# lucidrains/glom-pytorch

Hardware: NVIDIA H100
Metric: column-iterations/sec (BxNxLxiters) at dim=512 L=6 224/14 (higher is better)
Workload: dtype bf16

## Files before the change

### glom_pytorch_b200/csrc/engine.h

```cpp
#pragma once
#include <cuda.h>
#include <cuda_runtime.h>
#include <cuda_bf16.h>
#include <stdarg.h>
#include <stddef.h>
#include <stdint.h>
#include <stdio.h>
#include <atomic>
#include <mutex>
#include <vector>

#include "../../include/glom_b200.h"

namespace glom {

enum ProfKind { PROF_ATTN = 0, PROF_GEMM1 = 1, PROF_GEMM2 = 2, PROF_PREP = 3, PROF_TOKENIZE = 4, PROF_KINDS = 5 };
struct Profiler {
  bool enabled = false;
  std::vector<cudaEvent_t> ev;
  size_t used = 0;
  struct Span { int kind; size_t a, b; };
  std::vector<Span> spans;
  size_t mark(cudaStream_t st) {
    if (used == ev.size()) { cudaEvent_t e; cudaEventCreate(&e); ev.push_back(e); }
// ... 14 lines not shown
  int rows;
  int G;
  int hidden;
  int attend_self, mask_side, mask_d2_max;
  int bn2;
  int part_w;
  int nparts;
};

struct PackedLayout {
  size_t w1_off, w2_off, b1_off, b2_off, total;
};
PackedLayout packed_layout(int d, int L, int precision);

struct WorkspaceLayout {
  size_t s32_off;
  size_t s32_bytes;
  size_t sb_off[2];
  size_t sp_off[2];
  size_t xb_off;
  size_t h_off;
  size_t h_bytes;
  size_t c_off;
  size_t c_bytes;
  size_t nsq_off[2];
  size_t nsq_bytes;
  size_t attn_acc_off;
  size_t attn_acc_bytes;
  size_t total;
};
WorkspaceLayout workspace_layout(const Geometry& g, int precision, int iters, int return_all);

struct SettleLayout {
  WorkspaceLayout fwd;
  size_t dsq_off;
  size_t flags_off;
  size_t frozen_off;
  size_t block_frozen_off;
  size_t done_off;
  size_t level_q_off;
  size_t flags_bytes;
  size_t total;
};
SettleLayout settle_layout(const Geometry& g, int max_iters, int return_all = 0);

struct QueueLayout {
  SettleLayout settle;
  size_t slab_off[2];
  size_t queue_off;
  size_t slot_img_off;
  size_t age_off;
  size_t pending_off;
  size_t gather_off;
  size_t fresh_off;
  size_t block_fresh_off;
  size_t head_off;
  size_t unfinished_off;
  size_t queue_bytes;
  size_t total;
};
QueueLayout queue_layout(const Geometry& g, int max_iters);

struct QueueSlots {
  int *slot_img, *age, *pending, *gather_img, *fresh, *block_fresh, *head, *unfinished;
  int images, frames, max_iters;
};

struct Bf16Buffers {
  const float* s32_in;  float* s32_out;
  int s32_in_bcast;
  const __nv_bfloat16* sb_in;  __nv_bfloat16* sb_out;
  const __nv_bfloat16* sp_in;  __nv_bfloat16* sp_out;
  const __nv_bfloat16* xb;
  __nv_bfloat16* h;  __nv_bfloat16* c;
  float* attn_acc;
  const float* nsq_in;  float* nsq_out;
  const float* pos;
  const __nv_bfloat16* w1;  const __nv_bfloat16* w2;  const float* b1;  const float* b2;
  const int* frozen;
  const int* block_frozen;
  float* dsq_out;
  const int* block_fresh;
  int ii_reduce;
};

static inline int rep_h_blocks(int n) {
  int a = n, b = 128;
  while (b) { const int r = a % b; a = b; b = r; }
  return n / a;
}
static inline int rep_row_blocks(int n) { return (rep_h_blocks(n) * 128 + 255) / 256; }

typedef CUresult (*EncodeTiledFn)(CUtensorMap*, CUtensorMapDataType, cuuint32_t, void*, const cuuint64_t*,
                                  const cuuint64_t*, const cuuint32_t*, const cuuint32_t*, CUtensorMapInterleave,
                                  CUtensorMapSwizzle, CUtensorMapL2promotion, CUtensorMapFloatOOBfill);

struct Launch {
  EncodeTiledFn enc; int num_sms; cudaStream_t st; Profiler* prof;
  int launches;
  char err[400];
  int launched(cudaError_t e, const char* what = nullptr) { ++launches; return check(e, what); }
  int launched(const char* what = nullptr) { return launched(cudaGetLastError(), what); }
  int check(cudaError_t e, const char* what = nullptr) {
    if (e == cudaSuccess) return 0;
    return what ? fail(GLOM_B200_ERR_CUDA, "%s: %s", what, cudaGetErrorString(e)) : fail(GLOM_B200_ERR_CUDA, "%s", cudaGetErrorString(e));
  }
  int fail(int code, const char* fmt, ...) {
    char msg[sizeof(err)];
    va_list ap;
    va_start(ap, fmt);
    vsnprintf(msg, sizeof(msg), fmt, ap);
    va_end(ap);
    snprintf(err, sizeof(err), "%s", msg);
    return code;
  }
};
#define GLOM_TRY(x) do { if (const int r_ = (x)) return r_; } while (0)

int launch_prep(const Geometry& g, const float* state_in, const float* init_levels, const float* pos, const float* tokens,
                float* s32_dst, __nv_bfloat16* sb, __nv_bfloat16* sp, __nv_bfloat16* xb, float* nsq, Launch& ln);

int step_bf16(const Geometry& g, const Bf16Buffers& b, int step_index, Launch& ln);

int launch_settle_converge(const Geometry& g, int step, float tol, const float* dsq, const float* nsq, int* frozen,
                           int* block_frozen, unsigned int* done, float* level_q, int32_t* steps, Launch& ln,
                           const QueueSlots* q = nullptr);
int launch_queue_init(const Geometry& g, const QueueSlots& q, int* frozen, int* block_frozen, unsigned int* done, Launch& ln);
int launch_queue_schedule(const Geometry& g, const QueueSlots& q, int admit, int* frozen, int* block_frozen, Launch& ln);
int launch_queue_fill(const Geometry& g, const QueueSlots& q, const float* tokens, const float* pos, const float* state_in,
                      const float* init_levels, float* state_out, float* slab, __nv_bfloat16* sb, __nv_bfloat16* sp,
                      float* nsq, __nv_bfloat16* xb, Launch& ln);
int launch_settle_gather(const Geometry& g, int max_iters, const int32_t* steps, const float* slab, float* state_out,
                         const float* s0, int s0_bcast, Launch& ln);
int launch_steps_schedule(const Geometry& g, int t, int max_steps, const int32_t* steps, int* frozen, int* block_frozen,
                          Launch& ln);
int launch_steps_fill(const Geometry& g, int max_steps, const int32_t* steps, float* states, Launch& ln);
int launch_level_fill(const Geometry& g, float* states, Launch& ln);

constexpr int kAttnF32Queries = 16;
constexpr int kAttnF32MaxDimPlusN = (int)((227 * 1024) / (kAttnF32Queries * sizeof(float)));

struct F32Buffers {
  const float* s_in;  float* s_out;
  const float* x;  const float* pos;
  float* h;  float* c;
  const float* w1;  const float* w2;  const float* b1;  const float* b2;
};
int step_f32(const Geometry& g, const F32Buffers& b, Launch& ln);
int launch_broadcast_init(const Geometry& g, const float* state_in, const float* init_levels, float* dst, Launch& ln);

int launch_pack(int d, int L, int precision, const float* bu_w1, const float* bu_b1, const float* bu_w2, const float* bu_b2,
                const float* td_w1, const float* td_b1, const float* td_w2, const float* td_b2, void* packed, Launch& ln);

int launch_tokenize(const float* img, const float* w, const float* bias, float* tokens, int B, int H, int W, int p, int d,
                    Launch& ln);

int launch_islands(const float* states, int slabs, int side_h, int side_w, int L, int d, float threshold, float* cos_right,
                   float* cos_down, float* agreement, int* labels, int* num_islands, Launch& ln);
int launch_island_tree(const int* labels, const float* states, int slabs, int n, int L, int d, int* size, int* parent,
                       float* containment, float* nested, float* embedding, float* member_cos, float* coherence,
                       Launch& ln);

cudaError_t launch_clock_probe(unsigned long long* out, unsigned long long spin_ns, cudaStream_t st);
cudaError_t tc_kernel_clocks(unsigned long long* out , bool reset);

int launch_patchify_bf16(const float* img, const float* w, __nv_bfloat16* patches, __nv_bfloat16* wtok, int B, int H, int W,
// ... 106 lines not shown
```

### glom_pytorch_b200/csrc/gemm_sched.cuh

```cuda
#pragma once
#include "tc_common.cuh"

namespace glom {

struct GemmParams {
  int rows, d, L, n, G;
  int num_m, num_n, num_tiles;
  int m128;
  int z0;
  int n_half;
  const float* bias;
  const float* s32_in;
  int s_bcast;
  const __nv_bfloat16* c_in;
  const float* pos;
  float* s32_out;
  __nv_bfloat16* sb_out;
  __nv_bfloat16* sp_out;
  float* nsq_out;
  int nparts;
  float* tok_out;
  int tok_kb;
  const int* frozen;
  const int* block_frozen;
  float* dsq_out;
  const int* block_fresh;
  int num_m_rep, num_full_tiles;
  unsigned long long full_mask, rep_mask;
  int remap_l, h_period;
};

struct TileInfo {
  int z;
  int m_blk, n_blk;
  int num_kb;
};

__host__ __device__ __forceinline__ int nth_set_bit(unsigned long long m, int k) {
  int z = 0;
  for (;; ++z)
    if ((m >> z) & 1ull) { if (k == 0) return z; --k; }
}

template <int MODE, bool REDUCED = false>
__host__ __device__ __forceinline__ TileInfo decode_tile(const GemmParams& p, int tile) {
  TileInfo t;
  if (REDUCED && p.num_m_rep > 0) {
    const bool full = tile < p.num_full_tiles;
    const int nm = full ? p.num_m : p.num_m_rep;
    const int r = full ? tile / p.num_n : (tile - p.num_full_tiles) / p.num_n;
    t.n_blk = tile % p.num_n;
    t.m_blk = r % nm;
    t.z = nth_set_bit(full ? p.full_mask : p.rep_mask, r / nm);
  } else {
    t.n_blk = tile % p.num_n;
    const int r = tile / p.num_n;
    t.m_blk = r % p.num_m;
    t.z = p.z0 + r / p.num_m;
  }
  if (MODE == 0) t.num_kb = p.d / BK;
  else if (MODE == 1) t.num_kb = ((t.z == p.L - 1) ? 4 * p.d : 8 * p.d) / BK;
  else t.num_kb = p.tok_kb;
  return t;
}

template <int MODE>
__host__ __device__ __forceinline__ int sched_tile(const GemmParams& p, int c, int C, int it) {
  if (MODE != 1) { const int t = c + it * C; return t < p.num_tiles ? t : -1; }
  const int S = p.n_half;
  const int B = p.num_tiles - S;
  const int heavy = B % C;
  const int nb = (B - c + C - 1) / C;
  const int nbig = nb > 0 ? nb : 0;
  if (it < nbig) return c + it * C;
  int k = it - nbig;
  const int light = C - heavy;
  const int first = (2 * light < S) ? 2 * light : S;
  if (c >= heavy) {
    if (k < 2) { const int j = k * light + (c - heavy); if (j < first) return B + j; }
    k -= 2;
    if (k < 0) return -1;
  }
  const int j = first + k * C + c;
  return j < S ? B + j : -1;
}

__host__ __device__ __forceinline__ bool ii_k1_full(int z, int t) { return (z & 1) ? z <= 2 * t - 3 : z <= 2 * t; }
__host__ __device__ __forceinline__ bool ii_k2_full(int l, int t) { return l <= t; }
__host__ __device__ __forceinline__ int ii_k3_full_levels(int t) { return t; }

template <typename Full>
__host__ __forceinline__ void set_reduced(GemmParams& p, int z_end, int num_m_rep, Full full) {
  p.num_m_rep = num_m_rep;
  p.full_mask = p.rep_mask = 0;
  for (int z = p.z0; z < z_end; ++z) (full(z) ? p.full_mask : p.rep_mask) |= 1ull << z;
  p.num_full_tiles = __builtin_popcountll(p.full_mask) * p.num_m * p.num_n;
  p.num_tiles = p.num_full_tiles + __builtin_popcountll(p.rep_mask) * num_m_rep * p.num_n;
}

__host__ __device__ __forceinline__ void attn_item(int it, int full_items, int per_img, int ntiles, int l_full, int& b, int& l) {
  if (it >= full_items) { b = 0; l = l_full + (it - full_items) / ntiles; }
  else { b = it / per_img; l = (it % per_img) / ntiles; }
}

}
```

### glom_pytorch_b200/csrc/glom_api.cu

```cuda
#include "../../include/glom_b200.h"
#include "../../include/glom_b200_tree.h"
#include "engine.h"

#include <mutex>
#include <stdarg.h>
#include <stdio.h>
#include <string.h>

namespace glom {

static thread_local char g_err[512] = "";
static thread_local Profiler g_prof;
static thread_local Launch g_launch{};

static int fail(int code, const char* fmt, ...) {
  va_list ap;
  va_start(ap, fmt);
  vsnprintf(g_err, sizeof(g_err), fmt, ap);
  va_end(ap);
  return code;
}

static bool misaligned(const void* p, size_t a) { return reinterpret_cast<uintptr_t>(p) % a != 0; }

// ... 253 lines not shown
static void set_parity(StepBuffers& s, int p) {
  s.step.sb_in = s.sb[p]; s.step.sb_out = s.sb[p ^ 1];
  s.step.sp_in = s.sp[p]; s.step.sp_out = s.sp[p ^ 1];
  s.step.nsq_in = s.nsq[p]; s.step.nsq_out = s.nsq[p ^ 1];
}

struct SettleFlags { int *frozen, *block_frozen; float* dsq; unsigned int* done; float* level_q; };
static SettleFlags bind_settle_flags(const SettleLayout& sl, void* workspace) {
  char* ws = static_cast<char*>(workspace);
  return {reinterpret_cast<int*>(ws + sl.frozen_off), reinterpret_cast<int*>(ws + sl.block_frozen_off),
          reinterpret_cast<float*>(ws + sl.dsq_off), reinterpret_cast<unsigned int*>(ws + sl.done_off),
          reinterpret_cast<float*>(ws + sl.level_q_off)};
}

struct SettleRun { float tol; int32_t* steps; };

struct ForwardArgs {
  const glom_b200_cfg* cfg; const void* packed_weights; const float *tokens, *pos, *state_in, *init_levels; float* state_out;
  int batch, iters, return_all; void* workspace; size_t workspace_bytes; void* stream;
  int resume_parity = -1;
  const SettleRun* settle = nullptr;
  const int32_t* steps = nullptr;
};

static int forward_impl(const ForwardArgs& a) {
  const glom_b200_cfg* cfg = a.cfg;
  const float *state_in = a.state_in, *init_levels = a.init_levels;
  float* state_out = a.state_out;
  const int iters = a.iters, return_all = a.return_all;
  const SettleRun* settle = a.settle;
  const int32_t* steps = a.steps;
  if (int r = check_cfg(cfg)) return r;
  if (a.batch < 1 || iters < 0) return fail(GLOM_B200_ERR_INVALID, "batch must be >= 1 and iters >= 0");
  if (cfg->precision == GLOM_B200_FP32 && cfg->dim + cfg->n > kAttnF32MaxDimPlusN)
    return fail(GLOM_B200_ERR_INVALID,
                "fp32 consensus keeps %d (dim + n) floats per block in shared memory: dim + n must be <= %d (got %d)",
                kAttnF32Queries, kAttnF32MaxDimPlusN, cfg->dim + cfg->n);
  if (int r = check_tensors("", true, a.packed_weights, a.tokens, a.pos, state_in, init_levels, state_out, a.workspace)) return r;
  DeviceInfo di{};
  if (int r = device_info(&di)) return r;
  const Geometry g = make_geometry(cfg, a.batch);
  const bool freeze = settle || steps;
  const SettleLayout sl = freeze ? settle_layout(g, iters, return_all) : SettleLayout{};
  const WorkspaceLayout wl = freeze ? sl.fwd : workspace_layout(g, cfg->precision, iters, return_all);
  const size_t ws_need = freeze ? sl.total : wl.total;
  if (!a.workspace || a.workspace_bytes < ws_need)
    return fail(GLOM_B200_ERR_WORKSPACE, "workspace: need %zu bytes, got %zu", ws_need, a.workspace_bytes);
  const PackedLayout pl = packed_layout(g.d, g.L, cfg->precision);
  char* ws = static_cast<char*>(a.workspace);
  Launch& ln = begin_launch(di.sms, a.stream);
  const size_t slab = (size_t)g.rows * g.L * g.d;

  float* wslab = reinterpret_cast<float*>(ws + wl.s32_off);
  auto loc = [&](int t) -> float* {
    if (return_all) return state_out + (size_t)t * slab;
    return ((iters - t) % 2 == 0) ? state_out : wslab;
  };

  if (cfg->precision == GLOM_B200_BF16) {
    StepBuffers sbuf = bind_step_buffers(wl, pl, a.workspace, a.packed_weights, a.pos);
    Bf16Buffers& b = sbuf.step;
    const bool resume = a.resume_parity >= 0;
    const int p0 = resume ? a.resume_parity : 0;
    const bool s0_direct = resume || (!return_all && iters >= 1);
    int prep;
    if (resume) {
      prep = launch_prep(g, nullptr, nullptr, a.pos, a.tokens, nullptr, nullptr, nullptr, sbuf.xb, nullptr, ln);
      if (prep == 0 && return_all)
        prep = ln.launched(cudaMemcpyAsync(state_out, state_in, slab * sizeof(float), cudaMemcpyDeviceToDevice, ln.st));
    } else {
      prep = launch_prep(g, state_in, init_levels, a.pos, a.tokens, s0_direct ? nullptr : loc(0), sbuf.sb[0], sbuf.sp[0], sbuf.xb,
                         sbuf.nsq[0], ln);
    }
    if (prep) return fail(prep, "prep launch: %s", ln.err);
    const SettleFlags fl = freeze ? bind_settle_flags(sl, a.workspace) : SettleFlags{};
    b.frozen = fl.frozen; b.block_frozen = fl.block_frozen;
    b.dsq_out = settle ? fl.dsq : nullptr;
    if (settle) {
      if (int r = ln.check(cudaMemsetAsync(ws + sl.flags_off, 0, sl.flags_bytes, ln.st)))
        return fail(r, "settle flags memset: %s", ln.err);
    }
    const bool ii = !state_in && !resume && !freeze && iters >= g.L + 1 && g.L <= 32 &&
                    rep_row_blocks(g.n) < (g.rows + 255) / 256 && (size_t)g.n * g.L * g.d < (1u << 31);
    for (int t = 0; t < iters; ++t) {
      if (steps) {
        if (int r = launch_steps_schedule(g, t, iters, steps, fl.frozen, fl.block_frozen, ln))
          return fail(r, "step schedule launch before step %d: %s", t, ln.err);
      }
      b.s32_in = (s0_direct && t == 0) ? (state_in ? state_in : init_levels) : loc(t); b.s32_out = loc(t + 1);
      b.s32_in_bcast = (s0_direct && t == 0 && !state_in) ? 1 : 0;
      set_parity(sbuf, (t + p0) & 1);
      b.ii_reduce = ii && t < g.L;
      if (int r = step_bf16(g, b, t, ln)) return fail(r, "step %d: %s", t, ln.err);
      if (settle) {
        if (int r = launch_settle_converge(g, t + 1, settle->tol, fl.dsq, b.nsq_out, fl.frozen, fl.block_frozen, fl.done,
                                           fl.level_q, settle->steps, ln))
          return fail(r, "settle convergence launch after step %d: %s", t, ln.err);
      }
    }
    const int32_t* image_steps = settle ? settle->steps : steps;
    if (ii && return_all) {
      if (int r = launch_level_fill(g, state_out, ln)) return fail(r, "return_all level fill launch: %s", ln.err);
    }
    if (image_steps && return_all) {
      if (int r = launch_steps_fill(g, iters, image_steps, state_out, ln)) return fail(r, "return_all fill launch: %s", ln.err);
    } else if (image_steps && iters > 0) {
      if (int r = launch_settle_gather(g, iters, image_steps, wslab, state_out, state_in ? state_in : init_levels,
                                       state_in ? 0 : 1, ln))
        return fail(r, "%s gather launch: %s", settle ? "settle" : "step", ln.err);
    }
  } else {
    const char* pw = static_cast<const char*>(a.packed_weights);
    if (int r = launch_broadcast_init(g, state_in, init_levels, loc(0), ln)) return fail(r, "init launch: %s", ln.err);
    for (int t = 0; t < iters; ++t) {
      F32Buffers b{};
      b.s_in = loc(t); b.s_out = loc(t + 1);
      b.x = a.tokens; b.pos = a.pos;
      b.h = reinterpret_cast<float*>(ws + wl.h_off);
      b.c = reinterpret_cast<float*>(ws + wl.c_off);
      b.w1 = reinterpret_cast<const float*>(pw + pl.w1_off);
      b.w2 = reinterpret_cast<const float*>(pw + pl.w2_off);
      b.b1 = reinterpret_cast<const float*>(pw + pl.b1_off);
      b.b2 = reinterpret_cast<const float*>(pw + pl.b2_off);
      if (int r = step_f32(g, b, ln)) return fail(r, "fp32 step %d launch: %s", t, ln.err);
    }
  }
  g_err[0] = 0;
  return 0;
}

struct FreezeMode { const char* name; const char* bound; int min_bound; };
static const FreezeMode kSettle{"settle", "max_iters", 1}, kForwardSteps{"forward_steps", "max_steps", 0};

static int check_freeze(const FreezeMode& m, const glom_b200_cfg* cfg, int batch, int bound) {
  if (int r = check_cfg(cfg)) return r;
  if (cfg->precision != GLOM_B200_BF16) return fail(GLOM_B200_ERR_INVALID, "%s: bf16 engine only (precision fp32 given)", m.name);
  if (batch < 1) return fail(GLOM_B200_ERR_INVALID, "%s: batch must be >= 1 (got %d)", m.name, batch);
  if (bound < m.min_bound) return fail(GLOM_B200_ERR_INVALID, "%s: %s must be >= %d (got %d)", m.name, m.bound, m.min_bound, bound);
  return 0;
}

static int freeze_workspace_bytes(const FreezeMode& m, const glom_b200_cfg* cfg, int batch, int bound, int return_all,
                                  size_t* out_bytes) {
  if (int r = check_freeze(m, cfg, batch, bound)) return r;
  if (!out_bytes) return fail(GLOM_B200_ERR_INVALID, "out_bytes is NULL");
  *out_bytes = settle_layout(make_geometry(cfg, batch), bound, return_all ? 1 : 0).total;
  return 0;
}

static int check_steps_ptr(const char* fn, const char* arg, const int32_t* steps) {
  if (!steps) return fail(GLOM_B200_ERR_INVALID, "%s: %s is NULL", fn, arg);
  if (misaligned(steps, 4)) return fail(GLOM_B200_ERR_INVALID, "%s: %s must be 4-byte aligned", fn, arg);
  return 0;
}

static int settle_impl(ForwardArgs a, float tol, int32_t* steps_out) {
  if (int r = check_freeze(kSettle, a.cfg, a.batch, a.iters)) return r;
  if (tol != tol) return fail(GLOM_B200_ERR_INVALID, "settle: tol is NaN");
  if (int r = check_steps_ptr("settle", "steps_out", steps_out)) return r;
  const SettleRun run{tol, steps_out};
  a.settle = &run;
  return forward_impl(a);
}

GLOM_B200_API int glom_b200_settle_workspace_bytes(const glom_b200_cfg* cfg, int batch, int max_iters, size_t* out_bytes) {
  return freeze_workspace_bytes(kSettle, cfg, batch, max_iters, 0, out_bytes);
}

GLOM_B200_API int glom_b200_settle_workspace_offset(const glom_b200_cfg* cfg, int batch, int max_iters, int return_all,
                                                    int which, size_t* out_offset, size_t* out_bytes) {
  if (int r = check_freeze(kSettle, cfg, batch, max_iters)) return r;
  if (!out_offset || !out_bytes) return fail(GLOM_B200_ERR_INVALID, "settle: out_offset / out_bytes is NULL");
  const Geometry g = make_geometry(cfg, batch);
  const SettleLayout s = settle_layout(g, max_iters, return_all ? 1 : 0);
  switch (which) {
// ... 527 lines not shown
```

### glom_pytorch_b200/csrc/tc_kernels.cu

```cuda
#include "gemm_sched.cuh"
#include "tc_common.cuh"

#include <stdio.h>
#include <stdlib.h>
#include <string.h>

#include <type_traits>

namespace glom {

constexpr int GEMM_CONSUMER_WARPS = 8;
constexpr int GEMM_THREADS = 128 + 32 * GEMM_CONSUMER_WARPS;
constexpr uint32_t GEMM_PRODUCER_REGS = 40;
constexpr uint32_t GEMM_CONSUMER_REGS = 232;

__device__ unsigned long long g_kernel_clk[PROF_KINDS][8];


template <int MODE, int BN>
struct GemmCfg {
  static constexpr int PARTS = (BN == 256) ? 4 : 2;
  static constexpr int PART_COLS = BN / PARTS;
  static constexpr int THREADS = GEMM_THREADS;
  static constexpr uint32_t B_STAGE_BYTES = BN * BK * 2;
  static constexpr uint32_t STAGE_BYTES = A_STAGE_BYTES + B_STAGE_BYTES;
  static_assert(MODE >= 0 && MODE <= 2, "0 = GEMM1+GELU, 1 = GEMM2+combine, 2 = tokeniser");
  static constexpr int STAGES = (BN == 256) ? 3 : (BN == 128) ? 4 : 5;
  static constexpr uint32_t OUT_BOX_BYTES = 64 * BK * 2;
  static constexpr uint32_t PATCH_BYTES = 4096;
  static constexpr size_t EPI_BYTES = (MODE == 0) ? 2 * (BN / 64) * (size_t)OUT_BOX_BYTES
                                                  : 4 * (size_t)STG_BYTES + (size_t)GEMM_CONSUMER_WARPS * PATCH_BYTES + 4 * 32 * 4;
  static constexpr size_t SMEM_BYTES = 1024  + (size_t)STAGES * STAGE_BYTES + EPI_BYTES + 256 ;
  static_assert(SMEM_BYTES <= 232448, "over the 227 KB of shared memory a block may opt in to");
};

__device__ __forceinline__ void tok_chunk(const uint32_t (&v)[32], const float4 b4, uint8_t* patch, float* dst,
                                          size_t pitch, int lane, int rows_left) {
#pragma unroll
  for (int c = 0; c < 8; ++c)
    *reinterpret_cast<uint4*>(patch + lane * 128 + ((c ^ (lane & 7)) << 4)) =
        make_uint4(v[4 * c], v[4 * c + 1], v[4 * c + 2], v[4 * c + 3]);
  __syncwarp();
  const int c = lane & 7, rsub = lane >> 3;
#pragma unroll
  for (int i = 0; i < 8; ++i) {
    const int r = i * 4 + rsub;
    const float4 a = *reinterpret_cast<const float4*>(patch + r * 128 + ((c ^ (r & 7)) << 4));
    if (r < rows_left)
      *reinterpret_cast<float4*>(dst + (size_t)r * pitch + c * 4) = make_float4(a.x + b4.x, a.y + b4.y, a.z + b4.z, a.w + b4.w);
  }
  __syncwarp();
}

template <int MODE>
__device__ __forceinline__ bool settle_skip(const GemmParams& p, const TileInfo& t) {
  if (p.block_frozen[t.m_blk]) return true;
  return MODE == 0 && t.z == 0 && p.block_fresh != nullptr && !p.block_fresh[t.m_blk];
}

template <int MODE, int BN, bool CNT, bool SETTLE = false>
__global__ void __launch_bounds__(GEMM_THREADS, 1)
gemm_kernel(const __grid_constant__ CUtensorMap map_a0,
            const __grid_constant__ CUtensorMap map_a1,
            const __grid_constant__ CUtensorMap map_a2,
            const __grid_constant__ CUtensorMap map_b,
            const __grid_constant__ CUtensorMap map_out,
            const GemmParams p) {
  using Cfg = GemmCfg<MODE, BN>;
  constexpr int STAGES = Cfg::STAGES;
  constexpr bool RED = MODE != 2 && !SETTLE;
  extern __shared__ uint8_t smem_raw[];
  uint8_t* smem = smem_raw + ((1024u - (smem_u32(smem_raw) & 1023u)) & 1023u);
  uint8_t* epi = smem + (size_t)STAGES * Cfg::STAGE_BYTES;
  float* stg_all = reinterpret_cast<float*>(epi);
  uint8_t* patches = epi + 4 * STG_BYTES;
  float* xch = reinterpret_cast<float*>(patches + (size_t)GEMM_CONSUMER_WARPS * Cfg::PATCH_BYTES);
  uint64_t* full_bar = reinterpret_cast<uint64_t*>(epi + Cfg::EPI_BYTES);
  uint64_t* empty_bar = full_bar + STAGES;

  const int warp = threadIdx.x >> 5;
  const int lane = threadIdx.x & 31;
  constexpr int W_TMA = 0;
  constexpr int W_CONSUMER0 = 4;
  const int cta_rank = (int)(blockIdx.x & 1);
  const int cluster_id = blockIdx.x >> 1;
  const int num_clusters = gridDim.x >> 1;

  if (warp == W_TMA && lane == 0) {
    tma_prefetch_desc(&map_a0);
    tma_prefetch_desc(&map_b);
    if (MODE == 0) { tma_prefetch_desc(&map_a1); tma_prefetch_desc(&map_a2); tma_prefetch_desc(&map_out); }
    for (int i = 0; i < STAGES; ++i) { mbar_init(&full_bar[i], 1); mbar_init(&empty_bar[i], 2 * GEMM_CONSUMER_WARPS); }
    fence_barrier_init();
  }
  cluster_sync_all();
  pdl_launch_dependents();
  pdl_wait();
  const bool clk_thread = blockIdx.x == 0 && warp == W_TMA && lane == 0;
  ClockSample* clk_s = reinterpret_cast<ClockSample*>(empty_bar + STAGES);
  if (clk_thread) *clk_s = clock_sample_begin();
  const bool cnt_cta = CNT && blockIdx.x == 0;
  unsigned long long* const cnt = g_kernel_clk[MODE == 0 ? PROF_GEMM1 : MODE == 1 ? PROF_GEMM2 : PROF_TOKENIZE];
  unsigned long long w0 = 0, w1 = 0;
#define GLOM_CNT_WAIT(acc, stmt) do { if (cnt_cta) { const long long t_ = clock64(); stmt; acc += (unsigned long long)(clock64() - t_); } else { stmt; } } while (0)

  if (warp < W_CONSUMER0) {
    setmaxnreg_dec<GEMM_PRODUCER_REGS>();
    if (warp == W_TMA) {
      const uint32_t elected = elect_one();
      int stage = 0; uint32_t phase = 0;
      const uint32_t smem0 = smem_u32(smem);
      const uint64_t pol_first = l2_policy_evict_first();
      const int kbg_n = 4 * p.d / BK;
      const int blk_skip = (p.m128 - 1) * kbg_n;
      for (int it = 0, tile; (tile = sched_tile<MODE>(p, cluster_id, num_clusters, it)) >= 0; ++it) {
        const TileInfo t = decode_tile<MODE, RED>(p, tile);
        if constexpr (SETTLE) { if (settle_skip<MODE>(p, t)) continue; }
        const CUtensorMap* amap;
        int a_col, b_row;
        if (MODE == 0) {
          const int l = t.z >> 1;
          if (t.z == 0) { amap = &map_a0; a_col = 0; }
          else if (t.z & 1) { amap = &map_a2; a_col = l * p.d; }
          else { amap = &map_a1; a_col = (l - 1) * p.d; }
          b_row = t.z * 4 * p.d + t.n_blk * BN;
        } else if (MODE == 1) {
          amap = &map_a0; a_col = 0;
          b_row = t.z * p.d + t.n_blk * BN;
        } else {
          amap = &map_a0; a_col = 0;
          b_row = t.n_blk * BN;
        }
        const int a_row = t.m_blk * 256 + cta_rank * BM;
        const int blk0 = (2 * t.z * p.m128 + (a_row >> 7)) * kbg_n;
        int td_skip = blk_skip;
        if constexpr (RED && MODE == 1) {
          if (p.num_m_rep > 0 && t.z + 1 >= p.remap_l) td_skip -= ((a_row >> 7) - (a_row >> 7) % p.h_period) * kbg_n;
        }
        for (int kb = 0; kb < t.num_kb; ++kb) {
          GLOM_CNT_WAIT(w0, mbar_wait(&empty_bar[stage], phase ^ 1));
          if (elected) {
            const uint32_t sa = smem0 + (uint32_t)stage * Cfg::STAGE_BYTES;
            uint64_t* bar = &full_bar[stage];
            mbar_arrive_expect_tx(bar, Cfg::STAGE_BYTES);
            if (MODE == 1) {
              const int blk = blk0 + kb + (kb >= kbg_n ? td_skip : 0);
              tma_load_2d_hint(sa, amap, bar, 0, blk * BM, pol_first);
            } else {
              tma_load_2d(sa, amap, bar, a_col + kb * BK, a_row);
            }
            const uint32_t b_half = (uint32_t)cta_rank * (BN / 2);
            tma_load_2d_multicast(sa + A_STAGE_BYTES + b_half * BK * 2, &map_b, bar, kb * BK, b_row + (int)b_half, 0x3);
          }
          __syncwarp();
          if (++stage == STAGES) { stage = 0; phase ^= 1; }
        }
      }
      if (cnt_cta && elected) atomicAdd(&cnt[4], w0);
    }
  } else {
    setmaxnreg_inc<GEMM_CONSUMER_REGS>();
    const int cw = warp - W_CONSUMER0;
    const int wg = cw >> 2, wi = cw & 3;
    const int pair = cw >> 1, x = cw & 1;
    float* stg = stg_all + pair * (STG_BYTES / 4);
    uint8_t* patch = patches + (size_t)cw * Cfg::PATCH_BYTES;
    float* xch_p = xch + pair * 32;
    const uint32_t smem0 = smem_u32(smem);
    const uint64_t pol_stream = l2_policy_evict_first();
    const bool st_issuer = (threadIdx.x & 127) == 0;
    const uint32_t out_wg = smem_u32(epi) + (uint32_t)wg * (BN / 64) * Cfg::OUT_BOX_BYTES;
    const uint32_t st_row = (uint32_t)(16 * wi + 8 * ((lane >> 3) & 1) + (lane & 7)) * 128;
    const int st_jx = lane >> 4, st_sw = lane & 7;
    const uint32_t empty_peer = mapa_shared(smem_u32(empty_bar), (uint32_t)cta_rank ^ 1u);
    auto release = [&](int slot) {
      __syncwarp();
      if (lane == 0) { mbar_arrive(&empty_bar[slot]); mbar_arrive_cluster(empty_peer + 8u * (uint32_t)slot); }
    };
    int stage = 0; uint32_t phase = 0;
    float acc[BN / 2];
    for (int it = 0, tile; (tile = sched_tile<MODE>(p, cluster_id, num_clusters, it)) >= 0; ++it) {
      const TileInfo t = decode_tile<MODE, RED>(p, tile);
      if constexpr (SETTLE) { if (settle_skip<MODE>(p, t)) continue; }
      const int row0 = t.m_blk * 256 + cta_rank * BM + pair * 32;
      const int rows_left = p.rows - row0;
      uint32_t live = ~0u;
      if constexpr (SETTLE && MODE == 1)
        live = __ballot_sync(0xffffffffu, row0 + lane < p.rows && !p.frozen[(row0 + lane) / p.n]);
      bool remap = false;
      if constexpr (RED && MODE == 1) remap = p.num_m_rep > 0 && t.z >= p.remap_l;
      if (MODE == 1 && lane < rows_left) {
        const int src_row = remap ? (row0 + lane) % p.n : row0 + lane;
        const size_t o = ((size_t)src_row * p.L + t.z) * p.d + t.n_blk * BN + x * (BN / 2);
#pragma unroll
        for (int c = 0; c < BN / 2; c += 32) {
          if (!p.s_bcast) prefetch_l2(p.s32_in + o + c);
          if ((c & 63) == 0) prefetch_l2(p.c_in + o + c);
        }
      }
#pragma unroll
      for (int i = 0; i < BN / 2; ++i) acc[i] = 0.f;
      int prev = -1;
      for (int kb = 0; kb < t.num_kb; ++kb) {
        GLOM_CNT_WAIT(w0, mbar_wait(&full_bar[stage], phase));
        const uint32_t sa = smem0 + (uint32_t)stage * Cfg::STAGE_BYTES;
        wgmma_fence_regs(acc);
        wgmma_fence();
        wgmma_kblock<BN, 0>(acc, sa + (uint32_t)wg * (A_STAGE_BYTES / 2), sa + A_STAGE_BYTES);
        wgmma_commit();
        wgmma_wait<1>();
        wgmma_fence_regs(acc);
        if (prev >= 0) release(prev);
        prev = stage;
        if (++stage == STAGES) { stage = 0; phase ^= 1; }
      }
      wgmma_wait<0>();
      wgmma_fence_regs(acc);
      release(prev);
      const long long busy_t0 = cnt_cta ? clock64() : 0;
      if constexpr (MODE == 0) {
        const int wrow0 = t.m_blk * 256 + cta_rank * BM + 64 * wg;
        if (wrow0 < p.rows) {
          const int hblk0 = (t.z * p.m128 + (t.m_blk * 2 + cta_rank)) * (4 * p.d / BK) + t.n_blk * (BN / BK);
          const float* bias = p.bias + (size_t)t.z * 4 * p.d + t.n_blk * BN + 2 * (lane & 3);
          uint32_t pk[BN / 4];
#pragma unroll
          for (int s = 0; s < BN / 64; ++s) {
#pragma unroll
            for (int j = 0; j < 8; ++j) {
              const float2 b = __ldg(reinterpret_cast<const float2*>(bias + 64 * s + 8 * j));
#pragma unroll
              for (int h = 0; h < 2; ++h)
                pk[16 * s + 2 * j + h] = gelu_pair_bf16(acc[4 * (8 * s + j) + 2 * h], acc[4 * (8 * s + j) + 2 * h + 1], b.x, b.y);
            }
          }
          if (st_issuer) bulk_wait_group_read<0>();
          named_bar_sync(1 + wg, 128);
#pragma unroll
          for (int s = 0; s < BN / 64; ++s)
#pragma unroll
            for (int q = 0; q < 4; ++q)
              stmatrix_x4(out_wg + (uint32_t)s * Cfg::OUT_BOX_BYTES + st_row + ((uint32_t)((2 * q + st_jx) ^ st_sw) << 4),
                          pk[16 * s + 4 * q], pk[16 * s + 4 * q + 1], pk[16 * s + 4 * q + 2], pk[16 * s + 4 * q + 3]);
          fence_proxy_async_smem();
          named_bar_sync(1 + wg, 128);
          if (st_issuer) {
#pragma unroll
            for (int s = 0; s < BN / 64; ++s)
              tma_store_2d_hint(&map_out, out_wg + (uint32_t)s * Cfg::OUT_BOX_BYTES, 0, (hblk0 + s) * BM + 64 * wg, pol_stream);
            bulk_commit_group();
          }
        }
      } else {
#pragma unroll 1
        for (int s = 0; s < BN / 64; ++s) {
          stage_write(acc, stg, s, wi, lane);
          named_bar_sync(1 + pair, 64);
          uint32_t v[32];
          stage_read(stg, x, lane, v);
          const int cc = 64 * s + 32 * x;
          if (MODE == 2) {
            float* trow = p.tok_out + (size_t)row0 * p.d + t.n_blk * BN + cc;
            const float4 b4 = __ldg(reinterpret_cast<const float4*>(p.bias + t.n_blk * BN + cc + (lane & 7) * 4));
            tok_chunk(v, b4, patch, trow, (size_t)p.d, lane, rows_left);
          } else {
            K2Chunk kc;
            kc.l = t.z; kc.L = p.L; kc.d = p.d; kc.n = p.n; kc.row0 = row0; kc.prow0 = row0 % p.n; kc.s_bcast = p.s_bcast;
            kc.remap = remap;
            kc.s32_in = p.s32_in; kc.c_in = p.c_in; kc.pos = p.pos;
            kc.s32_out = p.s32_out; kc.sb_out = p.sb_out; kc.sp_out = p.sp_out;
            const int col = t.n_blk * BN + cc;
            const float4 b4 = __ldg(reinterpret_cast<const float4*>(p.bias + (size_t)t.z * p.d + col + (lane & 7) * 4));
            float rowsq[8], rowdsq[8];
#pragma unroll
            for (int i = 0; i < 8; ++i) rowsq[i] = rowdsq[i] = 0.f;
            const bool want_dsq = SETTLE && p.dsq_out != nullptr;
            if (rows_left >= 32) k2_chunk<true, SETTLE>(v, b4, patch, kc, col, lane, 32, rowsq, live, rowdsq, want_dsq);
            else k2_chunk<false, SETTLE>(v, b4, patch, kc, col, lane, rows_left, rowsq, live, rowdsq, want_dsq);
            int part = cc / Cfg::PART_COLS;
            bool writer = true;
            if (Cfg::PART_COLS == 64) {
              float* dxch = reinterpret_cast<float*>(patches + (size_t)(cw | 1) * Cfg::PATCH_BYTES);
              if (x == 1 && (lane & 7) == 0) {
#pragma unroll
                for (int i = 0; i < 8; ++i) xch_p[i * 4 + (lane >> 3)] = rowsq[i];
                if (want_dsq) {
#pragma unroll
                  for (int i = 0; i < 8; ++i) dxch[i * 4 + (lane >> 3)] = rowdsq[i];
                }
              }
              named_bar_sync(1 + pair, 64);
              if (x == 0) {
#pragma unroll
                for (int i = 0; i < 8; ++i) rowsq[i] += xch_p[i * 4 + (lane >> 3)];
                if (want_dsq) {
#pragma unroll
                  for (int i = 0; i < 8; ++i) rowdsq[i] += dxch[i * 4 + (lane >> 3)];
// ... 597 lines not shown
    AttnParams ap{};
    ap.n = n; ap.L = L; ap.d = d;
    ap.attend_self = g.attend_self; ap.mask_side = g.mask_side; ap.mask_d2_max = g.mask_d2_max;
    ap.key0 = npass == 1 ? 0 : pass * ATTN_PASS_KEYS;
    ap.nk = npass == 1 ? n : (n - ap.key0 < ATTN_PASS_KEYS ? n - ap.key0 : ATTN_PASS_KEYS);
    ap.pass_first = pass == 0; ap.pass_last = pass == npass - 1;
    ap.o_acc = b.attn_acc;
    ap.ml_acc = b.attn_acc ? b.attn_acc + (size_t)g.rows * L * d : nullptr;
    ap.n_pad16 = (ap.nk + 15) / 16 * 16;
    ap.n_pad64 = (ap.nk + 63) / 64 * 64;
    ap.nkb = (ap.n_pad16 + keys - 1) / keys;
    ap.nchunk = ap.n_pad64 / 64;
    ap.nparts = g.nparts;
    ap.nsq = b.nsq_in;
    ap.c_out = b.c;
    ap.scale = 1.0f / sqrtf((float)d);
    ap.ntiles = (n + BM - 1) / BM;
    ap.l_full = l_full;
    ap.num_items = ap.ntiles * (l_full * g.B + L - l_full);
    ap.frozen = b.frozen;
    const uint32_t slot = keys == 256 ? AttnCfg<256>::SLOT_BYTES : AttnCfg<128>::SLOT_BYTES;
    const size_t fixed = attn_fixed_smem(ap.nchunk, ap.n_pad16);
    const size_t max_smem = 232448;
    int stages = 4;
    while (stages > 0 && fixed + (size_t)stages * slot > max_smem) --stages;
    if (stages < 2 || ap.nkb > (keys == 256 ? AttnCfg<256>::MAX_KB : AttnCfg<128>::MAX_KB))
      return ln.fail(GLOM_B200_ERR_CUDA, "consensus pass of %d keys does not fit shared memory", ap.nk);
    ap.num_stages = stages;
    const size_t smem = fixed + (size_t)stages * slot;
    const int ctas = ap.num_items < ln.num_sms ? ap.num_items : ln.num_sms;
    ProfScope scope(ln.prof, PROF_ATTN, st);
    cudaError_t e;
    if (b.frozen) e = keys == 256 ? launch_attn_impl<256, false, true>(mq, mk, mv, ap, smem, ctas, st)
                                  : launch_attn_impl<128, false, true>(mq, mk, mv, ap, smem, ctas, st);
    else if (keys == 256) e = cnt ? launch_attn_impl<256, true>(mq, mk, mv, ap, smem, ctas, st)
                                          : launch_attn_impl<256, false>(mq, mk, mv, ap, smem, ctas, st);
    else e = cnt ? launch_attn_impl<128, true>(mq, mk, mv, ap, smem, ctas, st)
                         : launch_attn_impl<128, false>(mq, mk, mv, ap, smem, ctas, st);
    GLOM_TRY(ln.launched(e, "attn_kernel launch"));
  }
  return 0;
}

int step_bf16(const Geometry& g, const Bf16Buffers& b, int step_index, Launch& ln) {
  const int d = g.d, L = g.L, n = g.n, rows = g.rows, num_sms = ln.num_sms;
  cudaStream_t st = ln.st;
  CUtensorMap mh, mh_out;
  const int m128 = (rows + BM - 1) / BM;
  const uint64_t h_rows = (uint64_t)g.G * m128 * (4 * d / BK) * BM;
  GLOM_TRY(map2d(ln, &mh, b.h, h_rows, BK, BM, "H"));
  GLOM_TRY(map2d(ln, &mh_out, b.h, h_rows, BK, 64, "H out"));
  CUtensorMap mx, msb, msp, mw1, mw2;
  GLOM_TRY(map2d(ln, &mx, b.xb, rows, d, BM, "Xb"));
  GLOM_TRY(map2d(ln, &msb, b.sb_in, rows, (uint64_t)L * d, BM, "Sb"));
  GLOM_TRY(map2d(ln, &msp, b.sp_in, rows, (uint64_t)(L - 1) * d, BM, "Sp"));
  GLOM_TRY(map2d(ln, &mw1, b.w1, (uint64_t)g.G * 4 * d, d, 128, "W1p"));
  GLOM_TRY(map2d(ln, &mw2, b.w2, (uint64_t)L * d, (uint64_t)8 * d, (uint32_t)g.bn2 / 2, "W2p"));
  {
    GemmParams p{};
    p.rows = rows; p.d = d; p.L = L; p.n = n; p.G = g.G;
    p.z0 = (step_index > 0 && g.G > 1 && !b.block_fresh) ? 1 : 0;
    p.num_m = (rows + 255) / 256; p.num_n = 4 * d / 256; p.num_tiles = (g.G - p.z0) * p.num_m * p.num_n;
    p.bias = b.b1; p.m128 = m128;
    p.frozen = b.frozen; p.block_frozen = b.block_frozen; p.block_fresh = b.block_fresh;
    if (b.ii_reduce) set_reduced(p, g.G, rep_row_blocks(n), [&](int z) { return ii_k1_full(z, step_index); });
    ProfScope scope(ln.prof, PROF_GEMM1, st);
    GLOM_TRY(ln.launched(launch_gemm<0, 256>(mx, msb, msp, mw1, mh_out, p, num_sms, st), "gemm1 launch"));
  }
  GLOM_TRY(launch_attention(g, b, b.ii_reduce ? ii_k3_full_levels(step_index) : L, ln));
  {
    GemmParams p{};
    p.rows = rows; p.d = d; p.L = L; p.n = n; p.G = g.G;
    p.num_m = (rows + 255) / 256; p.num_n = d / g.bn2; p.z0 = 0; p.num_tiles = L * p.num_m * p.num_n;
    p.n_half = p.num_m * p.num_n;
    p.m128 = m128;
    p.bias = b.b2; p.s32_in = b.s32_in; p.s_bcast = b.s32_in_bcast; p.c_in = b.c; p.pos = b.pos;
    p.s32_out = b.s32_out; p.sb_out = b.sb_out; p.sp_out = b.sp_out; p.nsq_out = b.nsq_out; p.nparts = g.nparts;
    p.frozen = b.frozen; p.block_frozen = b.block_frozen; p.dsq_out = b.dsq_out;
    if (b.ii_reduce) {
      set_reduced(p, L, rep_row_blocks(n), [&](int l) { return ii_k2_full(l, step_index); });
      p.n_half = (L - 1 <= step_index ? p.num_m : p.num_m_rep) * p.num_n;
      p.remap_l = step_index; p.h_period = rep_h_blocks(n);
    }
    cudaError_t e;
    ProfScope scope(ln.prof, PROF_GEMM2, st);
    if (g.bn2 == 256) e = launch_gemm<1, 256>(mh, mh, mh, mw2, mh, p, num_sms, st);
    else if (g.bn2 == 128) e = launch_gemm<1, 128>(mh, mh, mh, mw2, mh, p, num_sms, st);
    else e = launch_gemm<1, 64>(mh, mh, mh, mw2, mh, p, num_sms, st);
    GLOM_TRY(ln.launched(e, "gemm2 launch"));
  }
  return 0;
}


int tokenize_tc(const __nv_bfloat16* patches, const __nv_bfloat16* wtok, const float* bias, float* tokens, int rows,
                int d, int kp, Launch& ln) {
  const int num_sms = ln.num_sms;
  cudaStream_t st = ln.st;
  const int bn = (d % 256 == 0) ? 256 : (d % 128 == 0) ? 128 : 64;
  CUtensorMap ma, mb;
  GLOM_TRY(map2d(ln, &ma, patches, rows, kp, BM, "patches"));
  GLOM_TRY(map2d(ln, &mb, wtok, d, kp, (uint32_t)bn / 2, "Wtok"));
  GemmParams p{};
  p.rows = rows; p.d = d; p.L = 1; p.n = 1; p.G = 1;
  p.num_m = (rows + 255) / 256; p.num_n = d / bn; p.num_tiles = p.num_m * p.num_n;
  p.bias = bias; p.tok_out = tokens; p.tok_kb = kp / BK;
  cudaError_t e;
  if (bn == 256) e = launch_gemm<2, 256>(ma, ma, ma, mb, ma, p, num_sms, st);
  else if (bn == 128) e = launch_gemm<2, 128>(ma, ma, ma, mb, ma, p, num_sms, st);
  else e = launch_gemm<2, 64>(ma, ma, ma, mb, ma, p, num_sms, st);
  return ln.launched(e, "tokeniser gemm launch");
}

}
```

Baseline: 68.12 million.

## Cache level-0 partial K2 product across iterations and skip its first K-segment

For level 0 of the second GEMM, the partial accumulator from the first K segment (4*d wide) is stored to fp32 scratch at step 0. At step 1 it is copied into the h buffer, and at later steps it is loaded to seed the accumulator so that segment's k-blocks are skipped. The level-0 tiles are also rescheduled into the light tail of the persistent tile order to rebalance work. This relies on that input segment staying constant across iterations after step 0. It adds fp32 loads and stores, and it reuses the h buffer as scratch, which risks aliasing.

```diff
diff --git a/glom_pytorch_b200/csrc/engine.h b/glom_pytorch_b200/csrc/engine.h
--- a/glom_pytorch_b200/csrc/engine.h
+++ b/glom_pytorch_b200/csrc/engine.h
@@ -120,6 +120,8 @@
   float* dsq_out;
   const int* block_fresh;
   int ii_reduce;
+  const float* p0_in;  float* p0_out;
+  int p0_in_ld, p0_out_ld;
 };
 
 static inline int rep_h_blocks(int n) {
diff --git a/glom_pytorch_b200/csrc/gemm_sched.cuh b/glom_pytorch_b200/csrc/gemm_sched.cuh
--- a/glom_pytorch_b200/csrc/gemm_sched.cuh
+++ b/glom_pytorch_b200/csrc/gemm_sched.cuh
@@ -28,6 +28,9 @@
   int num_m_rep, num_full_tiles;
   unsigned long long full_mask, rep_mask;
   int remap_l, h_period;
+  const float* p0_in;
+  float* p0_out;
+  int p0_in_ld, p0_out_ld, p0_tiles;
 };
 
 struct TileInfo {
@@ -85,6 +88,12 @@
   return j < S ? B + j : -1;
 }
 
+__host__ __device__ __forceinline__ int k2_tile(const GemmParams& p, int j) {
+  if (p.p0_tiles == 0) return j;
+  const int B = p.num_tiles - p.n_half;
+  return j < B ? j + p.p0_tiles : j < B + p.p0_tiles ? j - B : j;
+}
+
 __host__ __device__ __forceinline__ bool ii_k1_full(int z, int t) { return (z & 1) ? z <= 2 * t - 3 : z <= 2 * t; }
 __host__ __device__ __forceinline__ bool ii_k2_full(int l, int t) { return l <= t; }
 __host__ __device__ __forceinline__ int ii_k3_full_levels(int t) { return t; }
diff --git a/glom_pytorch_b200/csrc/glom_api.cu b/glom_pytorch_b200/csrc/glom_api.cu
--- a/glom_pytorch_b200/csrc/glom_api.cu
+++ b/glom_pytorch_b200/csrc/glom_api.cu
@@ -359,6 +359,8 @@
     }
     const bool ii = !state_in && !resume && !freeze && iters >= g.L + 1 && g.L <= 32 &&
                     rep_row_blocks(g.n) < (g.rows + 255) / 256 && (size_t)g.n * g.L * g.d < (1u << 31);
+    const bool l0 = !freeze && iters >= 2 && g.L >= 2;
+    float* const h_p0 = reinterpret_cast<float*>(b.h);
     for (int t = 0; t < iters; ++t) {
       if (steps) {
         if (int r = launch_steps_schedule(g, t, iters, steps, fl.frozen, fl.block_frozen, ln))
@@ -368,6 +370,13 @@
       b.s32_in_bcast = (s0_direct && t == 0 && !state_in) ? 1 : 0;
       set_parity(sbuf, (t + p0) & 1);
       b.ii_reduce = ii && t < g.L;
+      if (l0) {
+        const int ld_slab = g.L * g.d;
+        b.p0_in = t == 0 ? nullptr : t == 1 ? loc(2) : h_p0;
+        b.p0_in_ld = t == 1 ? ld_slab : g.d;
+        b.p0_out = t == 0 ? loc(2) : t == 1 ? h_p0 : nullptr;
+        b.p0_out_ld = t == 0 ? ld_slab : g.d;
+      }
       if (int r = step_bf16(g, b, t, ln)) return fail(r, "step %d: %s", t, ln.err);
       if (settle) {
         if (int r = launch_settle_converge(g, t + 1, settle->tol, fl.dsq, b.nsq_out, fl.frozen, fl.block_frozen, fl.done,
diff --git a/glom_pytorch_b200/csrc/tc_kernels.cu b/glom_pytorch_b200/csrc/tc_kernels.cu
--- a/glom_pytorch_b200/csrc/tc_kernels.cu
+++ b/glom_pytorch_b200/csrc/tc_kernels.cu
@@ -50,6 +50,32 @@
       *reinterpret_cast<float4*>(dst + (size_t)r * pitch + c * 4) = make_float4(a.x + b4.x, a.y + b4.y, a.z + b4.z, a.w + b4.w);
   }
   __syncwarp();
+}
+
+template <int BN>
+__device__ __forceinline__ void p0_store(const float (&acc)[BN / 2], float* p, int ld, int row, int rows) {
+#pragma unroll
+  for (int h = 0; h < 2; ++h) {
+    if (row + 8 * h >= rows) continue;
+    float* r = p + (size_t)(row + 8 * h) * ld;
+#pragma unroll
+    for (int j = 0; j < BN / 8; ++j)
+      *reinterpret_cast<float2*>(r + 8 * j) = make_float2(acc[4 * j + 2 * h], acc[4 * j + 2 * h + 1]);
+  }
+}
+template <int BN>
+__device__ __forceinline__ void p0_load(float (&acc)[BN / 2], bool on, const float* p, int ld, int row, int rows) {
+#pragma unroll
+  for (int h = 0; h < 2; ++h) {
+    const bool ok = on && row + 8 * h < rows;
+    const float* r = p + (size_t)(ok ? row + 8 * h : 0) * ld;
+#pragma unroll
+    for (int j = 0; j < BN / 8; ++j) {
+      const float2 v = ok ? *reinterpret_cast<const float2*>(r + 8 * j) : make_float2(0.f, 0.f);
+      acc[4 * j + 2 * h] = v.x;
+      acc[4 * j + 2 * h + 1] = v.y;
+    }
+  }
 }
 
 template <int MODE>
@@ -114,7 +140,7 @@
       const int kbg_n = 4 * p.d / BK;
       const int blk_skip = (p.m128 - 1) * kbg_n;
       for (int it = 0, tile; (tile = sched_tile<MODE>(p, cluster_id, num_clusters, it)) >= 0; ++it) {
-        const TileInfo t = decode_tile<MODE, RED>(p, tile);
+        const TileInfo t = decode_tile<MODE, RED>(p, (RED && MODE == 1) ? k2_tile(p, tile) : tile);
         if constexpr (SETTLE) { if (settle_skip<MODE>(p, t)) continue; }
         const CUtensorMap* amap;
         int a_col, b_row;
@@ -137,7 +163,9 @@
         if constexpr (RED && MODE == 1) {
           if (p.num_m_rep > 0 && t.z + 1 >= p.remap_l) td_skip -= ((a_row >> 7) - (a_row >> 7) % p.h_period) * kbg_n;
         }
-        for (int kb = 0; kb < t.num_kb; ++kb) {
+        int kb0 = 0;
+        if constexpr (RED && MODE == 1) { if (p.p0_in && t.z == 0) kb0 = kbg_n; }
+        for (int kb = kb0; kb < t.num_kb; ++kb) {
           GLOM_CNT_WAIT(w0, mbar_wait(&empty_bar[stage], phase ^ 1));
           if (elected) {
             const uint32_t sa = smem0 + (uint32_t)stage * Cfg::STAGE_BYTES;
@@ -180,7 +208,7 @@
     int stage = 0; uint32_t phase = 0;
     float acc[BN / 2];
     for (int it = 0, tile; (tile = sched_tile<MODE>(p, cluster_id, num_clusters, it)) >= 0; ++it) {
-      const TileInfo t = decode_tile<MODE, RED>(p, tile);
+      const TileInfo t = decode_tile<MODE, RED>(p, (RED && MODE == 1) ? k2_tile(p, tile) : tile);
       if constexpr (SETTLE) { if (settle_skip<MODE>(p, t)) continue; }
       const int row0 = t.m_blk * 256 + cta_rank * BM + pair * 32;
       const int rows_left = p.rows - row0;
@@ -198,10 +226,15 @@
           if ((c & 63) == 0) prefetch_l2(p.c_in + o + c);
         }
       }
-#pragma unroll
-      for (int i = 0; i < BN / 2; ++i) acc[i] = 0.f;
+      const int kbg_n = 4 * p.d / BK;
+      bool seeded = false, p0_keep = false;
+      if constexpr (RED && MODE == 1) { seeded = p.p0_in && t.z == 0; p0_keep = p.p0_out && t.z == 0; }
+      const int p0_row = t.m_blk * 256 + cta_rank * BM + 64 * wg + 16 * wi + (lane >> 2);
+      const int p0_col = t.n_blk * BN + 2 * (lane & 3);
+      p0_load<BN>(acc, seeded, p.p0_in + p0_col, p.p0_in_ld, p0_row, p.rows);
+      if (seeded && p0_keep) p0_store<BN>(acc, p.p0_out + p0_col, p.p0_out_ld, p0_row, p.rows);
       int prev = -1;
-      for (int kb = 0; kb < t.num_kb; ++kb) {
+      for (int kb = seeded ? kbg_n : 0; kb < t.num_kb; ++kb) {
         GLOM_CNT_WAIT(w0, mbar_wait(&full_bar[stage], phase));
         const uint32_t sa = smem0 + (uint32_t)stage * Cfg::STAGE_BYTES;
         wgmma_fence_regs(acc);
@@ -213,6 +246,11 @@
         if (prev >= 0) release(prev);
         prev = stage;
         if (++stage == STAGES) { stage = 0; phase ^= 1; }
+        if (p0_keep && !seeded && kb == kbg_n - 1) {
+          wgmma_wait<0>();
+          wgmma_fence_regs(acc);
+          p0_store<BN>(acc, p.p0_out + p0_col, p.p0_out_ld, p0_row, p.rows);
+        }
       }
       wgmma_wait<0>();
       wgmma_fence_regs(acc);
@@ -976,6 +1014,10 @@
       p.n_half = (L - 1 <= step_index ? p.num_m : p.num_m_rep) * p.num_n;
       p.remap_l = step_index; p.h_period = rep_h_blocks(n);
     }
+    if ((b.p0_in || b.p0_out) && (b.block_frozen || L < 2))
+      return ln.fail(GLOM_B200_ERR_INVALID, "level-0 product needs the default K2 build and L >= 2");
+    p.p0_in = b.p0_in; p.p0_out = b.p0_out; p.p0_in_ld = b.p0_in_ld; p.p0_out_ld = b.p0_out_ld;
+    if (b.p0_in) { p.p0_tiles = p.num_m * p.num_n; p.n_half += p.p0_tiles; }
     cudaError_t e;
     ProfScope scope(ln.prof, PROF_GEMM2, st);
     if (g.bn2 == 256) e = launch_gemm<1, 256>(mh, mh, mh, mw2, mh, p, num_sms, st);
```

Result: faster. 69.49 million, median of 6 (+2.0%).
